# utiasASRL/mm_masking

Measured on AMD Instinct MI355X. Metric: scan-pairs/s (mask-CNN + 10-iter dICP fwd+bwd), higher is better.
Workload: dtype bf16; 1 GPU; BASELINE configs[2]: train_icp_weights step fwd+bwd, batch=32 per GPU, 10 dICP iters, point-to-plane Huber, dim=2; 400x3360 polar radar -> GO-CFAR + peaks + polar->Cartesian 640x640 -> U-Net (hand-written NHWC bf16 MFMA kernels, fp32 masters) -> dICP (fp32 points, fp64 normal equations) -> rot+trans+mask_pts loss -> Adam; batch_per_gpu=32, global_batch=32, scan_pts_pad=5120, map_pts=20000, map_pts_pad=20480, icp_iters=10, parallelism=dp1, scene_density=survey (SURVEY.md 8d: 3 500-5 000 valid scan points of 5 120)

## Files before the change

mm_masking_amd/csrc/mmk_unet.hip:

```cpp
#include <math.h>
#include <stdlib.h>

#include <algorithm>
#include <type_traits>

#include "mmk_common.h"
#include "mmk_unet_shared.h"

namespace {

using namespace mmku;

__device__ __forceinline__ unsigned cvt_pk_bf16(float lo, float hi)
{
    unsigned r;
    asm("v_cvt_pk_bf16_f32 %0, %1, %2" : "=v"(r) : "v"(lo), "v"(hi));
    return r;
}
__device__ __forceinline__ unsigned pk_relu_bf16(unsigned x)
{
    unsigned r;
    asm("v_pk_max_i16 %0, %1, 0" : "=v"(r) : "v"(x));
    return r;
}
// ... 670 lines not shown

    float bs8[8];
    if constexpr (C8) {
#pragma unroll
        for (int r = 0; r < 8; ++r) {
            bs8[r] = a.bias ? a.bias[r] : 0.f;
            asm volatile("" : "+v"(bs8[r]));
        }
    }
    const float dk = dp.inv_keep;
    const unsigned thr1pk = ((unsigned)(dp.thr_s - 1 < -32768 ? -32768 : dp.thr_s - 1) & 0xffffu) * 0x00010001u;
#pragma unroll
    for (int m = 0; m < MT; ++m)
#pragma unroll
        for (int r = 0; r < 4; ++r) bs[m][r] *= dk;
    if constexpr (C8) {
#pragma unroll
        for (int r = 0; r < 8; ++r) bs8[r] *= dk;
    }

    MMK_RING_LOAD(0);
    MMK_RING_LOAD(1);
    MMK_RING_SINKS();
    if constexpr (RD > 2) {
        MMK_RING_LOAD(2);
        MMK_RING_SINKS();
    }
    cur_pix0 = s_pix0[0]; cur_ty0 = s_ty0[0]; cur_tx0 = s_tx0[0];
    if constexpr (POOL) cur_pp0 = s_pp0[0];
    MMK_RING_STORE(0, 0);
    MMK_RING_LOAD(0);
    MMK_RING_SINKS();

    int k0 = 0;
    {
#define STAGE_CHECKED 1
#define STAGE_SLOT 0
#include "mmk_conv_ring_stage.inc"
#undef STAGE_SLOT
#define STAGE_SLOT 1
#include "mmk_conv_ring_stage.inc"
#undef STAGE_SLOT
        if constexpr (RD > 2) {
#define STAGE_SLOT 2
#include "mmk_conv_ring_stage.inc"
#undef STAGE_SLOT
        }
#undef STAGE_CHECKED
    }
    for (k0 = RD; k0 + RD <= nt_blk; k0 += RD) {
#define STAGE_CHECKED 0
#define STAGE_SLOT 0
#include "mmk_conv_ring_stage.inc"
#undef STAGE_SLOT
#define STAGE_SLOT 1
#include "mmk_conv_ring_stage.inc"
#undef STAGE_SLOT
        if constexpr (RD > 2) {
#define STAGE_SLOT 2
#include "mmk_conv_ring_stage.inc"
#undef STAGE_SLOT
        }
#undef STAGE_CHECKED
    }
    {
#define STAGE_CHECKED 1
#define STAGE_SLOT 0
#include "mmk_conv_ring_stage.inc"
#undef STAGE_SLOT
        if constexpr (RD > 2) {
#define STAGE_SLOT 1
#include "mmk_conv_ring_stage.inc"
#undef STAGE_SLOT
        }
#undef STAGE_CHECKED
    }
ring_done:;
#ifdef MMK_DEEP_STAMPS
    if (tid == 0) { stamp_lds[16 + 6] = __builtin_amdgcn_s_memtime(); stamp_lds[16 + 7] = __builtin_amdgcn_s_memrealtime(); }
    __syncthreads();
    if (g_deep_stamp_buf != nullptr && blockIdx.y == 0 && blockIdx.x < 4096 && tid == 0) {
        unsigned long long *life = g_deep_stamp_buf + (size_t)64 * (4 * MMK_STAMP_STAGES * 8) + (size_t)blockIdx.x * 2;
        life[0] = stamp_lds[8 + 7];
        life[1] = stamp_lds[16 + 7];
    }
    if (g_deep_stamp_buf != nullptr && blockIdx.y == 0 && blockIdx.x < 64)
        for (int i = tid; i < 4 * MMK_STAMP_STAGES * 8; i += CONV_THREADS)
            g_deep_stamp_buf[(size_t)blockIdx.x * (4 * MMK_STAMP_STAGES * 8) + i] = stamp_lds[i];
#endif
#undef MMK_RING_LOAD
#undef MMK_RING_STORE
}

template <int CK, int CM, int RD, bool EPI, int POOL = 0, bool C8 = false, bool POOLG = false>
int launch_conv_ring(const ConvArgs &a, hipStream_t st)
{
#ifdef MMK_DEEP_STAMPS
    const size_t smem = (((size_t)2 * HT * WT * lds_pitch(CK) + (size_t)ksteps(CK) * (CM / 16) * 512) * sizeof(bf16) + 15) / 16 * 16 +
                        (size_t)4 * MMK_STAMP_STAGES * 8 * sizeof(unsigned long long);
#else
    const size_t smem = ((size_t)2 * HT * WT * lds_pitch(CK) + (size_t)ksteps(CK) * (CM / 16) * 512) * sizeof(bf16);
#endif
    constexpr auto kernel = conv3x3_ring_kernel<CK, CM, RD, EPI, POOL, C8, POOLG>;
    int per_cu = 0;
    MMK_CHECK_HIP(blocks_per_cu<kernel>(CONV_THREADS, smem, 8, &per_cu));
    const int groups = (a.COUT + CM - 1) / CM;
    const XcdGrid g = xcd_grid(a.B, a.H, a.W, TH, TW, groups, per_cu);
    hipLaunchKernelGGL(kernel, dim3(8 * g.nb, groups), dim3(CONV_THREADS), smem, st, a, g.total, g.per_xcd);
    MMK_LAUNCH_CHECK();
    return MMK_OK;
}

inline bool use_c8_epilogue()
{
    static int v = -1;
    if (v < 0) {
        const char *e = getenv("MMK_CONV_C8");
        v = (e && e[0] == '0') ? 0 : 1;
    }
    return v == 1;
}

template <int CK, int CM>
int launch_conv_ring_epi(const ConvArgs &a, hipStream_t st)
{
    constexpr int RD = CK <= 16 ? 3 : 2;
    constexpr int RDE = 2;
    const bool epi = a.o1.relu_src || a.o1.accumulate || (a.o2.C > 0 && (a.o2.relu_src || a.o2.accumulate));
    if (a.x1_pool_arg != nullptr) {
        if constexpr (CK == 32 && CM == 32) {
            if (epi && a.pool_y == nullptr) return launch_conv_ring<CK, CM, RDE, true, 0, false, true>(a, st);
        }
        mmk::set_error("mmk_conv3x3: x1_pool_arg is not supported for this layer (CIN=%d COUT=%d)", a.CIN, a.COUT);
        return MMK_ERR_ARG;
    }
    if (a.pool_y != nullptr) {
        if constexpr (CK == CM && (CK == 16 || CK == 32)) {
            if (!epi && a.o2.C == 0)
                return a.pool_arg != nullptr ? launch_conv_ring<CK, CM, RD, false, 2>(a, st) : launch_conv_ring<CK, CM, RD, false, 1>(a, st);
        }
        mmk::set_error("mmk_conv3x3: pool_y is not supported for this layer (see mmk_conv3x3_pool_fusable)");
        return MMK_ERR_ARG;
    }
    if constexpr (CM == 16) {
        if (a.COUT == 8 && a.o2.C == 0 && use_c8_epilogue())
            return epi ? launch_conv_ring<CK, CM, RDE, true, false, true>(a, st) : launch_conv_ring<CK, CM, RD, false, false, true>(a, st);
    }
    return epi ? launch_conv_ring<CK, CM, RDE, true>(a, st) : launch_conv_ring<CK, CM, RD, false>(a, st);
}


constexpr int DEEP_THREADS = 512;

template <int BM, int NT>
struct DeepCfg {
    static constexpr int WM = BM >= 128 ? 2 : 1;
    static constexpr int WN = 8 / WM;
    static constexpr int MT = BM / 16 / WM;
    static constexpr int MTB = BM / 16;
    static constexpr int TH = WN, TWD = NT * 16;
    static constexpr int HT = TH + 2, WT = TWD + 2;
    static constexpr int CK = 32, PK = 48, NS = 9, GPP = 4;
    static constexpr int NIN = HT * WT * GPP;
    static constexpr int NW = NS * MTB * 64;
    static constexpr int RIN = (NIN + DEEP_THREADS - 1) / DEEP_THREADS;
    static constexpr int RW = (NW + DEEP_THREADS - 1) / DEEP_THREADS;
    static constexpr size_t IN_BYTES = (size_t)HT * WT * PK * sizeof(bf16), W_BYTES = (size_t)NW * 8 * sizeof(bf16);
    static constexpr size_t smem_core(int wchunks) { return IN_BYTES + (size_t)wchunks * W_BYTES + BM * sizeof(float); }
#ifdef MMK_DEEP_STAMPS
    static constexpr size_t smem(int wchunks) { return (smem_core(wchunks) + 15) / 16 * 16 + (size_t)8 * MMK_STAMP_STAGES * 8 * sizeof(unsigned long long); }
#else
    static constexpr size_t smem(int wchunks) { return smem_core(wchunks); }
#endif
};

template <int BM, int NT>
XcdGrid deep_grid(int B, int H, int W, int cout)
{
    return xcd_grid(B, H, W, DeepCfg<BM, NT>::TH, DeepCfg<BM, NT>::TWD, (cout + BM - 1) / BM, 1);
}

template <int BM, int NT, bool LK = false, bool SUBW = false, int ROLE = 0, bool WRES = false, bool POOLG = false>
__global__ __launch_bounds__(DEEP_THREADS) void conv3x3_deep_kernel(const ConvArgs a, int total_tiles, int tiles_per_xcd)
{
    using C = DeepCfg<BM, NT>;
    constexpr int MT = C::MT, MTB = C::MTB, PK = C::PK, WT = C::WT, HT = C::HT, GPP = C::GPP;
    constexpr int NIN = C::NIN, NW = C::NW, RIN = C::RIN, RW = C::RW, NS = C::NS;
    constexpr bool R_FWD = ROLE == 1, R_BWD = ROLE == 2;
    static_assert(!(WRES && SUBW), "resident weights: the kernel's own packing only");
    extern __shared__ __attribute__((aligned(16))) unsigned char smem[];
    bf16 *in_tile = reinterpret_cast<bf16 *>(smem);
    bf16 *w_lds = in_tile + HT * WT * PK;

    const int tid = threadIdx.x, lane = tid & 63, wv = tid >> 6;
    const int wm = wv / C::WN, wn = wv % C::WN;
    const int tiles_x = (a.W + C::TWD - 1) / C::TWD, tiles_y = (a.H + C::TH - 1) / C::TH;
    const int tpi = tiles_x * tiles_y;
    const int group = blockIdx.y;
    const int nchunk = a.CIN / 32;
    const int wchunks = WRES ? nchunk : 1;

    const int xcd = blockIdx.x & 7, nb = gridDim.x >> 3;
    const int t_begin = xcd * tiles_per_xcd;
    const int t_end = (t_begin + tiles_per_xcd < total_tiles) ? t_begin + tiles_per_xcd : total_tiles;
    int tile = t_begin + (blockIdx.x >> 3);
    if (tile >= t_end) return;

    constexpr int RWL = WRES ? 0 : RW;
    constexpr int PHT = C::TH / 2 + 2, PWT = C::TWD / 2 + 2, NPIN = PHT * PWT * GPP;
    constexpr int NRIN = POOLG ? (NPIN + DEEP_THREADS - 1) / DEEP_THREADS : RIN;
    u32x4 rin[NRIN], rw[RW];
    unsigned rcd[POOLG ? NRIN : 1];
    const int Hp = a.H >> 1, Wp = a.W >> 1;
    int g_dy[RIN], g_dx[RIN], g_c[RIN], g_pix[RIN];
#pragma unroll
    for (int i = 0; i < RIN; ++i) {
        int g = tid + i * DEEP_THREADS;
        g = g < NIN ? g : NIN - 1;
        const int pix = g / GPP;
        g_dy[i] = pix / WT - 1;
        g_dx[i] = pix % WT - 1;
        g_c[i] = (g % GPP) * 8;
        g_pix[i] = (pix / WT) * a.W + pix % WT;
        if constexpr (POOLG) {
            int gp = tid + i * DEEP_THREADS;
            gp = gp < NPIN ? gp : NPIN - 1;
            const int pp = gp / GPP;
            g_dy[i] = pp / PWT - 1;
            g_dx[i] = pp % PWT - 1;
            g_c[i] = (gp % GPP) * 8;
            g_pix[i] = g_dy[i] * Wp + g_dx[i];
        }
    }
    const bf16 *ld_base = nullptr;
    int ld_xc = 0, ld_ty0 = 0, ld_tx0 = 0;
    const u32x4 *ld_w = nullptr;
    const unsigned *ld_code = nullptr;
    int ld_moff = 0;
    auto set_stage = [&](int t, int chunk) {
        const int b = t / tpi, tr = t - b * tpi;
        const int tyi = tr / tiles_x;
        ld_tx0 = (tr - tyi * tiles_x) * C::TWD;
        ld_ty0 = tyi * C::TH;
        const int c0 = chunk * 32;
        const bool in1 = c0 < a.C1;
        const bf16 *xb = in1 ? a.x1 : a.x2;
        ld_xc = in1 ? a.C1 : a.C2;
        const int cb = in1 ? c0 : c0 - a.C1;
        const long org = POOLG ? ((long)b * Hp + (ld_ty0 >> 1)) * Wp + (ld_tx0 >> 1)
                               : ((long)b * a.H + ld_ty0 - 1) * a.W + ld_tx0 - 1;
        ld_base = xb + org * ld_xc + cb;
        if constexpr (POOLG) ld_code = a.x1_pool_arg + ((org * ld_xc + cb) >> 3);
        if constexpr (SUBW) {
            const int pm = a.wpack_mtb, per = pm / MTB;
            ld_w = reinterpret_cast<const u32x4 *>(a.wpack + ((size_t)((group / per) * nchunk + chunk)) * NS * pm * 512);
            ld_moff = (group % per) * MTB;
        } else {
            ld_w = reinterpret_cast<const u32x4 *>(a.wpack + ((size_t)(group * nchunk + chunk)) * NW * 8);
        }
    };
    auto issue_in = [&](int i) {
        if constexpr (POOLG) {
            const bool ok = (unsigned)((ld_ty0 >> 1) + g_dy[i]) < (unsigned)Hp && (unsigned)((ld_tx0 >> 1) + g_dx[i]) < (unsigned)Wp;
            const int off = g_pix[i] * ld_xc + g_c[i];
            rin[i] = *(ok ? reinterpret_cast<const u32x4 *>(ld_base + off) : &g_zero16);
            rcd[i] = *(ok ? ld_code + (off >> 3) : reinterpret_cast<const unsigned *>(&g_zero16));
            return;
        }
        const bool ok = (unsigned)(ld_ty0 + g_dy[i]) < (unsigned)a.H && (unsigned)(ld_tx0 + g_dx[i]) < (unsigned)a.W;
        const unsigned off = (unsigned)(g_pix[i] * ld_xc + g_c[i]);
        const u32x4 *sp = ok ? reinterpret_cast<const u32x4 *>(ld_base + off) : &g_zero16;
        rin[i] = *sp;
    };
    auto issue_w = [&](int i) {
        int g = tid + i * DEEP_THREADS;
        g = g < NW ? g : NW - 1;
        if constexpr (SUBW) rw[i] = ld_w[((g / (MTB * 64)) * a.wpack_mtb + ld_moff) * 64 + g % (MTB * 64)];
        else rw[i] = ld_w[g];
    };
    auto write_in = [&]() {
        if constexpr (POOLG) {
#pragma unroll
            for (int i = 0; i < NRIN; ++i) {
                const int g = tid + i * DEEP_THREADS;
                const int r0 = 2 * g_dy[i] + 1, c0 = 2 * g_dx[i] + 1;
                poolg_write(in_tile + (r0 * WT + c0) * PK + g_c[i], PK, WT * PK, r0, c0, HT, WT, g < NPIN, rin[i], rcd[i], a.x1_pool_scale);
            }
            return;
        }
#pragma unroll
        for (int i = 0; i < RIN; ++i) {
            const int g = tid + i * DEEP_THREADS;
            if (g < NIN) *reinterpret_cast<u32x4 *>(in_tile + (size_t)(g / GPP) * PK + (g % GPP) * 8) = rin[i];
        }
    };
    auto write_w = [&](int slot) {
#pragma unroll
        for (int i = 0; i < RW; ++i) {
            const int g = tid + i * DEEP_THREADS;
            if (g < NW) reinterpret_cast<u32x4 *>(w_lds + (size_t)slot * NW * 8)[g] = rw[i];
        }
    };

    const DropoutParams dp = dropout_params(a.drop_p);
    float *bias_lds = reinterpret_cast<float *>(w_lds + (size_t)wchunks * NW * 8);
    if (tid < BM) {
        int c = group * BM + tid;
        if constexpr (SUBW) {
            const int pm = a.wpack_mtb, per = pm / MTB, m_off = (group % per) * MTB;
            c = (group / per) * (pm * 16) + (m_off / 4) * 64 + 16 * (tid / (4 * MT)) + 4 * (m_off % 4) + tid % (4 * MT);
        }
        const float bz = (a.bias && c < a.COUT) ? a.bias[c] : 0.f;
        bias_lds[tid] = R_FWD ? bz * dp.inv_keep : bz;
    }
    f32x4 acc[MT][NT];
    auto reset_acc = [&]() {
#pragma unroll
        for (int m = 0; m < MT; ++m)
#pragma unroll
            for (int n = 0; n < NT; ++n) acc[m][n] = f32x4{0.f, 0.f, 0.f, 0.f};
    };
    reset_acc();

    constexpr bool lk = LK;
    const bf16 *b_base = in_tile + ((size_t)(wn * WT + (lane & 15))) * PK + 8 * (lane >> 4);
    const bf16 *a_base0 = w_lds + ((size_t)(wm * MT) * 64 + lane) * 8;

    int chunk = 0;
#ifdef MMK_DEEP_STAMPS
    unsigned long long *stamp_lds = reinterpret_cast<unsigned long long *>(smem + (C::smem_core(wchunks) + 15) / 16 * 16);
    int stamp_stage = 0;
    for (int i = tid; i < 8 * MMK_STAMP_STAGES * 8; i += DEEP_THREADS) stamp_lds[i] = 0ull;
#endif
    if constexpr (WRES) {
        for (int ck = 0; ck < nchunk; ++ck) {
            set_stage(tile, ck);
#pragma unroll
            for (int i = 0; i < RW; ++i) issue_w(i);
            write_w(ck);
        }
    }
    set_stage(tile, 0);
#pragma unroll
    for (int i = 0; i < NRIN; ++i) issue_in(i);
    if constexpr (!WRES) {
#pragma unroll
        for (int i = 0; i < RW; ++i) issue_w(i);
        write_w(0);
    }
    write_in();
    __syncthreads();

    constexpr int NCH = 4 * MT;
    constexpr int LW = NCH >= 8 ? 8 : 4;
    typedef __attribute__((ext_vector_type(LW))) __bf16 bfl;
    constexpr int NP = NCH / LW;

    while (true) {
        MMK_STAMP(0);
        int ntile = tile, nck = chunk + 1;
        if (nck == nchunk) {
            nck = 0;
            ntile = tile + nb;
        }
        const bool has_next = ntile < t_end;
        set_stage(has_next ? ntile : tile, nck);
        const bf16 *a_base = a_base0 + (WRES ? (size_t)chunk * NW * 8 : (size_t)0);
        MMK_STAMP(1);
#pragma unroll
        for (int s = 0; s < NS; ++s) {
            const int ty = s / 3, tx = s % 3;
            bf16x8 bf[NT];
#pragma unroll
            for (int n = 0; n < NT; ++n)
                bf[n] = *reinterpret_cast<const bf16x8 *>(b_base + ((size_t)(ty * WT + n * 16 + tx)) * PK);
#pragma unroll
            for (int m = 0; m < MT; ++m) {
                const bf16x8 af = *reinterpret_cast<const bf16x8 *>(a_base + ((size_t)(s * MTB + m) * 64) * 8);
#pragma unroll
                for (int n = 0; n < NT; ++n) acc[m][n] = __builtin_amdgcn_mfma_f32_16x16x32_bf16(af, bf[n], acc[m][n], 0, 0, 0);
            }
#pragma unroll
            for (int j = s; j < NRIN + RWL; j += NS) {
                if (j < NRIN) issue_in(j);
                else issue_w(j - NRIN);
            }
            __builtin_amdgcn_sched_barrier(0x38F);
        }
        MMK_STAMP(2);
        auto deliver_and_write = [&]() {
#pragma unroll
            for (int i = 0; i < NRIN; ++i) asm volatile("" : "+v"(rin[i]));
            if constexpr (POOLG) {
#pragma unroll
                for (int i = 0; i < NRIN; ++i) asm volatile("" : "+v"(rcd[i]));
            }
#pragma unroll
            for (int i = 0; i < RWL; ++i) asm volatile("" : "+v"(rw[i]));
            MMK_STAMP(4);
            if (has_next) {
                __syncthreads();
                MMK_STAMP(5);
                write_in();
                if constexpr (!WRES) write_w(0);
            }
            MMK_STAMP(6);
        };
        if (chunk != nchunk - 1) {
            MMK_STAMP(3);
            deliver_and_write();
        } else {
            const int b = tile / tpi, tr = tile - b * tpi;
            const int tyi = tr / tiles_x;
            const int tx0 = (tr - tyi * tiles_x) * C::TWD, yy = tyi * C::TH + wn;
            int lv = lane;
            asm volatile("" : "+v"(lv));
            const int g4 = lv >> 4;
            int c0, e_bias_at;
            if constexpr (SUBW) {
                const int pm = a.wpack_mtb, per = pm / MTB, m_off = (group % per) * MTB;
                c0 = (group / per) * (pm * 16) + (m_off / 4) * 64 + 16 * g4 + 4 * (m_off % 4);
                e_bias_at = NCH * g4;
            } else {
                c0 = group * BM + wm * (16 * MT) + NCH * g4;
                e_bias_at = wm * (16 * MT) + NCH * g4;
            }
            const bool e_on = c0 < a.COUT;
            const bool firstp = c0 < a.o1.C;
            bf16 *const o_y = firstp ? a.o1.y : a.o2.y;
            const bf16 *const o_src = firstp ? a.o1.relu_src : a.o2.relu_src;
            const int o_C = firstp ? a.o1.C : a.o2.C;
            const bool e_acc = (firstp ? a.o1.accumulate : a.o2.accumulate) != 0;
            const float e_scale = firstp ? a.o1.scale : a.o2.scale;
            const int cl = firstp ? c0 : c0 - a.o1.C;
            const int e_x0 = tx0 + (lv & 15);
            const long p0 = ((long)b * a.H + yy) * a.W + e_x0;
            const unsigned e_e0 = (unsigned)p0 * (unsigned)a.COUT + (unsigned)c0 + a.hash_base;
            bf16 *const e_y0 = o_y + p0 * o_C + cl;
            const int e_step = 16 * o_C;
            const bool e_row_ok = yy < a.H;
            const bool e_src = o_src != nullptr;
            const bf16 *const e_pf0 = e_src ? o_src + p0 * o_C + cl : (e_acc ? (const bf16 *)e_y0 : nullptr);
            bfl opnd[R_BWD ? NT : 1][NP];
            auto fetch_operands = [&]() {
#pragma unroll
                for (int n = 0; n < NT; ++n) {
                    const bool okp = e_on && e_pf0 != nullptr && e_row_ok && e_x0 + n * 16 < a.W;
                    const bf16 *pp = okp ? e_pf0 + n * e_step : reinterpret_cast<const bf16 *>(g_zero32);
#pragma unroll
                    for (int k = 0; k < NP; ++k) opnd[R_BWD ? n : 0][k] = *reinterpret_cast<const bfl *>(pp + k * LW);
                }
            };
            if constexpr (R_BWD) fetch_operands();
            if (e_on) {
                if constexpr (R_FWD) {
                    float bk[NCH];
#pragma unroll
                    for (int k = 0; k < NCH; k += 4) {
                        const f32x4 t = *reinterpret_cast<const f32x4 *>(bias_lds + e_bias_at + k);
                        bk[k] = t[0]; bk[k + 1] = t[1]; bk[k + 2] = t[2]; bk[k + 3] = t[3];
                    }
                    const float kf = dp.inv_keep;
                    const int t1s = (int)dp.thr - 32768 - 1;
                    const unsigned t1 = (unsigned)(t1s < -32768 ? -32768 : t1s) & 0xffffu;
                    const unsigned thr1 = t1 | (t1 << 16);
                    const bool drop = dp.thr != 0u;
#pragma unroll
                    for (int n = 0; n < NT; ++n) {
                        const bool okp = e_row_ok && e_x0 + n * 16 < a.W;
                        unsigned hw[MT][2];
#pragma unroll
                        for (int m = 0; m < MT; ++m) hw[m][0] = hw[m][1] = 0x7fff7fffu;
                        if (drop) {
#pragma unroll
                            for (int m = 0; m < MT; ++m)
                                dropout_words(a.seed, e_e0 + (unsigned)n * (16u * (unsigned)a.COUT) + 4u * m, hw[m][0], hw[m][1]);
                        }
                        unsigned pk[NCH / 2];
#pragma unroll
                        for (int m = 0; m < MT; ++m)
#pragma unroll
                            for (int hlf = 0; hlf < 2; ++hlf) {
                                const float t0 = __builtin_fmaf(acc[m][n][2 * hlf], kf, bk[4 * m + 2 * hlf]);
                                const float t1f = __builtin_fmaf(acc[m][n][2 * hlf + 1], kf, bk[4 * m + 2 * hlf + 1]);
                                pk[2 * m + hlf] = pk_relu_bf16(cvt_pk_bf16(t0, t1f)) & pk_keep_mask(hw[m][hlf], thr1);
                            }
                        bf16 *const dst = okp ? e_y0 + n * e_step : reinterpret_cast<bf16 *>(g_sink32);
                        if constexpr (NCH >= 8) {
#pragma unroll
                            for (int k = 0; k < NCH / 2; k += 4)
                                *reinterpret_cast<u32x4 *>(dst + 2 * k) = (u32x4){pk[k], pk[k + 1], pk[k + 2], pk[k + 3]};
                        } else {
                            *reinterpret_cast<unsigned long long *>(dst) = ((unsigned long long)pk[1] << 32) | pk[0];
                        }
                        __builtin_amdgcn_sched_barrier(0);
                    }
                } else {
                    float bv[NCH];
                    if constexpr (!R_BWD) {
#pragma unroll
                        for (int k = 0; k < NCH; k += 4) {
                            const f32x4 t = *reinterpret_cast<const f32x4 *>(bias_lds + e_bias_at + k);
                            bv[k] = t[0]; bv[k + 1] = t[1]; bv[k + 2] = t[2]; bv[k + 3] = t[3];
                        }
                    }
                    const bool o_accf = !e_src && e_acc;
#pragma unroll
                    for (int n = 0; n < NT; ++n) {
                        const bool okp = e_row_ok && e_x0 + n * 16 < a.W;
                        float v[NCH];
#pragma unroll
                        for (int m = 0; m < MT; ++m)
#pragma unroll
                            for (int r = 0; r < 4; ++r) {
                                float t = acc[m][n][r];
                                if constexpr (!R_BWD) {
                                    t += bv[4 * m + r];
                                    if (a.relu) t = lk ? act_leaky(t, a.slope) : fmaxf(t, 0.f);
                                }
                                v[4 * m + r] = t;
                            }
                        if constexpr (!R_BWD) {
                            if (dp.thr != 0u) {
#pragma unroll
                                for (int m = 0; m < MT; ++m) {
                                    float sc[4];
                                    dropout_scale4(a.seed, e_e0 + (unsigned)n * (16u * (unsigned)a.COUT) + 4u * m, dp, sc);
#pragma unroll
                                    for (int r = 0; r < 4; ++r) v[4 * m + r] = lk ? drop_leaky(v[4 * m + r], sc[r]) : v[4 * m + r] * sc[r];
                                }
                            }
                        }
                        bf16 *const dst0 = e_y0 + n * e_step;
                        if constexpr (R_BWD) {
                            if (e_pf0 != nullptr && okp) {
                                if (!o_accf) {
#pragma unroll
                                    for (int k = 0; k < NCH; k += LW) {
                                        const bfl sv = opnd[n][k / LW];
#pragma unroll
                                        for (int r = 0; r < LW; ++r) v[k + r] = ((float)sv[r] > 0.f) ? v[k + r] * e_scale : 0.f;
                                    }
                                } else {
#pragma unroll
                                    for (int k = 0; k < NCH; k += LW) {
                                        const bfl ov = opnd[n][k / LW];
#pragma unroll
                                        for (int r = 0; r < LW; ++r) v[k + r] += (float)ov[r];
                                    }
                                }
                            }
                        } else {
                            if (e_src && okp) {
                                const bf16 *sp = e_pf0 + n * e_step;
#pragma unroll
                                for (int k = 0; k < NCH; k += LW) {
                                    const bfl sv = *reinterpret_cast<const bfl *>(sp + k);
#pragma unroll
                                    for (int r = 0; r < LW; ++r)
                                        v[k + r] = lk ? v[k + r] * bwd_factor_leaky((float)sv[r], e_scale, a.slope)
                                                      : (((float)sv[r] > 0.f) ? v[k + r] * e_scale : 0.f);
                                }
                            }
                            if (e_acc && okp) {
#pragma unroll
                                for (int k = 0; k < NCH; k += LW) {
                                    const bfl ov = *reinterpret_cast<const bfl *>(dst0 + k);
#pragma unroll
                                    for (int r = 0; r < LW; ++r) v[k + r] += (float)ov[r];
                                }
                            }
                        }
                        if (R_BWD || okp) {
                            bf16 *const dst = (R_BWD && !okp) ? reinterpret_cast<bf16 *>(g_sink32) : dst0;
                            if constexpr (NCH >= 8) {
#pragma unroll
                                for (int k = 0; k < NCH; k += 8) {
                                    bf16x8 o8;
#pragma unroll
                                    for (int r = 0; r < 8; ++r) o8[r] = (bf16)v[k + r];
                                    *reinterpret_cast<bf16x8 *>(dst + k) = o8;
                                }
                            } else {
                                bf16x4 o4;
#pragma unroll
                                for (int r = 0; r < 4; ++r) o4[r] = (bf16)v[r];
                                *reinterpret_cast<bf16x4 *>(dst) = o4;
                            }
                        }
                    }
                }
            }
            reset_acc();
            MMK_STAMP(3);
            deliver_and_write();
        }
        if (!has_next) break;
        __syncthreads();
        MMK_STAMP(7);
#ifdef MMK_DEEP_STAMPS
        ++stamp_stage;
#endif
        tile = ntile;
        chunk = nck;
    }
#ifdef MMK_DEEP_STAMPS
    __syncthreads();
    if (g_deep_stamp_buf != nullptr && blockIdx.y == 0 && blockIdx.x < 64)
        for (int i = tid; i < 8 * MMK_STAMP_STAGES * 8; i += DEEP_THREADS)
            g_deep_stamp_buf[(size_t)blockIdx.x * (8 * MMK_STAMP_STAGES * 8) + i] = stamp_lds[i];
#endif
}

template <int BM, int NT, bool LK = false, bool SUBW = false, int ROLE = 0, bool WRES = false, bool POOLG = false>
int launch_conv_deep(const ConvArgs &a, hipStream_t st)
{
    using C = DeepCfg<BM, NT>;
    constexpr auto kernel = conv3x3_deep_kernel<BM, NT, LK, SUBW, ROLE, WRES, POOLG>;
    MMK_CHECK_HIP(raise_lds_limit<kernel>(true, 160 * 1024));
    const size_t smem = C::smem(WRES ? a.CIN / 32 : 1);
    MMK_REQUIRE(smem <= (size_t)160 * 1024, "mmk_conv3x3: %zu bytes of LDS for CIN=%d COUT=%d", smem, a.CIN, a.COUT);
    const XcdGrid g = deep_grid<BM, NT>(a.B, a.H, a.W, a.COUT);
    hipLaunchKernelGGL(kernel, dim3(8 * g.nb, (a.COUT + BM - 1) / BM), dim3(DEEP_THREADS), smem, st, a, g.total, g.per_xcd);
    MMK_LAUNCH_CHECK();
    return MMK_OK;
}

template <int BM, int NT>
bool deep_weights_fit(int cin) { return DeepCfg<BM, NT>::smem(cin / 32) <= (size_t)160 * 1024; }

template <class F>
int with_deep_cfg(int BM, bool narrow, F &&f)
{
    return with_int<16, 32, 64, 128>(BM, [&](auto M) {
        return narrow ? f(M, std::integral_constant<int, 3>{}) : f(M, std::integral_constant<int, 5>{});
    });
}

int deep_rounds(int B, int H, int W, int cout, int BM, bool narrow, int *tiles_per_image)
{
    return with_deep_cfg(BM, narrow, [&](auto M, auto NT) {
        const XcdGrid g = deep_grid<M(), NT()>(B, H, W, cout);
        if (tiles_per_image) *tiles_per_image = g.tiles;
        return g.rounds();
    });
}

int dispatch_conv_deep_plain(const ConvArgs &a, hipStream_t st);

int dispatch_conv_deep(const ConvArgs &a, hipStream_t st)
{
    const int BM = conv_cm(a.CIN, a.COUT);
    const bool narrow = a.W <= 48;
    const char *split_env = getenv("MMK_CONV_SPLIT");
    const bool split_on = !(split_env && split_env[0] == '0');
    int tpi = 0;
    const bool forward_role = a.relu != 0 && a.o1.relu_src == nullptr && a.o2.relu_src == nullptr && !a.o1.accumulate && !a.o2.accumulate;
    if (split_on && forward_role && a.slope == 0.f && (BM == 64 || BM == 128) && a.COUT % 32 == 0 && a.pool_y == nullptr && a.wpack_mtb == 0 &&
        deep_rounds(a.B, a.H, a.W, a.COUT, BM, narrow, &tpi) == 2) {
        const int groups = (a.COUT + BM - 1) / BM, nb = std::max(1, 32 / groups);
        const int Bm = (8 * nb) / tpi;
        const int Bt = a.B - Bm;
        const bool under_filled = (long)a.B * tpi * groups * 10 < (long)256 * 2 * 7;
        if (Bm >= 1 && Bt >= 1 && under_filled && deep_rounds(Bm, a.H, a.W, a.COUT, BM, narrow, nullptr) == 1 &&
            deep_rounds(Bt, a.H, a.W, a.COUT, 32, narrow, nullptr) == 1 && (a.o1.C % 32 == 0) && (a.o2.C % 32 == 0)) {
            ConvArgs m = a;
            m.B = Bm;
            int rc = dispatch_conv_deep_plain(m, st);
            if (rc != MMK_OK) return rc;
            ConvArgs t = a;
            const size_t px = (size_t)Bm * a.H * a.W;
            t.B = Bt;
            t.x1 = a.x1 + px * a.C1;
            if (a.x2) t.x2 = a.x2 + px * a.C2;
            auto adv = [&](ConvOutPart &o) {
                if (o.y) o.y += px * o.C;
                if (o.relu_src) o.relu_src += px * o.C;
            };
            adv(t.o1);
            adv(t.o2);
            t.hash_base = a.hash_base + (unsigned)(px * a.COUT);
            t.wpack_mtb = BM / 16;
            return narrow ? launch_conv_deep<32, 3, false, true, 1>(t, st) : launch_conv_deep<32, 5, false, true, 1>(t, st);
        }
    }
    return dispatch_conv_deep_plain(a, st);
}

int dispatch_conv_deep_plain(const ConvArgs &a, hipStream_t st)
{
    const bool any_src = a.o1.relu_src != nullptr || (a.o2.C > 0 && a.o2.relu_src != nullptr);
    const bool any_acc = a.o1.accumulate != 0 || (a.o2.C > 0 && a.o2.accumulate != 0);
    const bool both1 = a.o1.relu_src != nullptr && a.o1.accumulate != 0, both2 = a.o2.C > 0 && a.o2.relu_src != nullptr && a.o2.accumulate != 0;
    const int role = (a.relu != 0 && !any_src && !any_acc) ? 1
                   : ((a.relu == 0 && a.bias == nullptr && dropout_params(a.drop_p).thr == 0u && !both1 && !both2) ? 2 : 0);
    const int rc = with_deep_cfg(conv_cm(a.CIN, a.COUT), a.W <= 48, [&](auto M, auto N) -> int {
        constexpr int BM = M(), NT = N();
        constexpr bool WRES = BM <= 64;
        const bool resident = WRES && a.wpack_mtb == 0 && deep_weights_fit<BM, NT>(a.CIN);
        if (a.slope > 0.f) return launch_conv_deep<BM, NT, true>(a, st);
        if (a.x1_pool_arg != nullptr) {
            if constexpr (BM >= 64) {
                if (role == 2 && a.wpack_mtb == 0) {
                    if (resident) return launch_conv_deep<BM, NT, false, false, 2, WRES, true>(a, st);
                    if (BM > 64) return launch_conv_deep<BM, NT, false, false, 2, false, true>(a, st);
                }
            }
            mmk::set_error("mmk_conv3x3: x1_pool_arg is not supported for this layer (CIN=%d COUT=%d)", a.CIN, a.COUT);
            return MMK_ERR_ARG;
        }
        if constexpr (BM >= 32) {
            if (role == 1) return resident ? launch_conv_deep<BM, NT, false, false, 1, WRES>(a, st) : launch_conv_deep<BM, NT, false, false, 1>(a, st);
            if (role == 2) return resident ? launch_conv_deep<BM, NT, false, false, 2, WRES>(a, st) : launch_conv_deep<BM, NT, false, false, 2>(a, st);
        }
        return launch_conv_deep<BM, NT>(a, st);
    });
    if (rc != NO_KERNEL) return rc;
    mmk::set_error("mmk_conv3x3: unsupported channel counts CIN=%d COUT=%d", a.CIN, a.COUT);
    return MMK_ERR_ARG;
}

bool pool_fusable(int cin, int cout, int B, int H, int W)
{
    const bool fits32 = (size_t)B * H * W * (size_t)std::max(cin, cout) < ((size_t)1 << 31);
    return cin == cout && (cin == 16 || cin == 32) && fits32 && H >= 2 && W >= 2;
}

template <class F>
int with_thin_shape(int CK, int CM, F &&f)
{
    return with_int<8, 16, 32>(CK, [&](auto K) {
        return with_int<16, 32, 64>(CM, [&](auto M) {
            if constexpr (K() == 32 && M() == 64) return NO_KERNEL;
            else return f(K, M);
        });
    });
}

int dispatch_conv(const ConvArgs &a, hipStream_t st)
{
    if (a.pool_y != nullptr && (a.slope > 0.f || !pool_fusable(a.CIN, a.COUT, a.B, a.H, a.W))) {
        mmk::set_error("mmk_conv3x3: pool_y is not supported for this layer (see mmk_conv3x3_pool_fusable)");
        return MMK_ERR_ARG;
    }
    if (a.x1_pool_arg != nullptr && (a.slope > 0.f || a.C2 != 0 || a.H < 2 || a.W < 2)) {
        mmk::set_error("mmk_conv3x3: x1_pool_arg needs the ReLU network, a single input and H, W >= 2");
        return MMK_ERR_ARG;
    }
    if (conv_is_deep(a.CIN, a.COUT)) {
        if (a.o2.C > 0 && conv_cm(a.CIN, a.COUT) >= 64 && a.o1.C % 16 != 0) {
            mmk::set_error("mmk_conv3x3: output split %d+%d: layers of >= 64 output channels split at multiples of 16", a.o1.C, a.o2.C);
            return MMK_ERR_ARG;
        }
        return dispatch_conv_deep(a, st);
    }
    const int CK = conv_ck(a.CIN), CM = conv_cm(a.CIN, a.COUT);
    if (a.x1_pool_arg != nullptr && !(a.CIN == 32 && CM == 32 && (size_t)a.B * a.H * a.W * 32 < ((size_t)1 << 31))) {
        mmk::set_error("mmk_conv3x3: x1_pool_arg is not supported for this layer (CIN=%d COUT=%d)", a.CIN, a.COUT);
        return MMK_ERR_ARG;
    }
    const bool fits32 = (size_t)a.B * a.H * a.W * (size_t)std::max(a.CIN, a.COUT) < ((size_t)1 << 31);
    const bool ring = a.CIN == CK && CM <= 32 && fits32;
    const int rc = with_thin_shape(CK, CM, [&](auto K, auto M) -> int {
        if (a.slope > 0.f) return launch_conv<K(), M(), true>(a, st);
        if constexpr (M() <= 32) {
            if (ring) return launch_conv_ring_epi<K(), M()>(a, st);
        }
        return launch_conv<K(), M()>(a, st);
    });
    if (rc != NO_KERNEL) return rc;
    mmk::set_error("mmk_conv3x3: unsupported channel counts CIN=%d COUT=%d", a.CIN, a.COUT);
    return MMK_ERR_ARG;
}


typedef __attribute__((ext_vector_type(2))) int i32x2;
typedef __attribute__((ext_vector_type(4))) int i32x4;

__device__ __forceinline__ unsigned lds_addr(const void *p)
{
    return (unsigned)(size_t)(__attribute__((address_space(3))) const void *)p;
}

__device__ __forceinline__ i32x2 tr_read(unsigned addr)
{
    i32x2 v;
    asm volatile("ds_read_b64_tr_b16 %0, %1" : "=v"(v) : "v"(addr) : "memory");
    return v;
}

template <int OFF>
__device__ __forceinline__ i32x2 tr_read_o(unsigned addr)
{
    static_assert(OFF >= 0 && OFF < 65536, "ds offset field is 16 bits");
    i32x2 v;
    asm volatile("ds_read_b64_tr_b16 %0, %1 offset:%2" : "=v"(v) : "v"(addr), "n"(OFF) : "memory");
    return v;
}

__device__ __forceinline__ bf16x8 frag_from(i32x2 lo, i32x2 hi)
{
    i32x4 t = {lo.x, lo.y, hi.x, hi.y};
    return __builtin_bit_cast(bf16x8, t);
}

struct WgradArgs {
    const bf16 *x1, *x2;
    int C1, C2;
    const bf16 *g;
    int B, H, W, CIN, COUT;
    float *partials;
    int acc_partials;
    const unsigned *g_arg = nullptr;
    float g_scale = 1.f;
};

template <int CK, int CM, bool G8, bool POOLG = false>
__global__ __launch_bounds__(CONV_THREADS) void conv3x3_wgrad_kernel(const WgradArgs a)
{
    constexpr int MT = CM / 16;
    constexpr int NTT = (CK >= 16) ? 9 * (CK / 16) : 5;
    constexpr int NTW = (NTT + 3) / 4;
    extern __shared__ __attribute__((aligned(16))) unsigned char smem[];
    constexpr int PK = wg_pitch(CK);
    constexpr int GCOLS = G8 ? 8 : CM;
    constexpr int PG = wg_pitch(GCOLS);
    bf16 *x_tile = reinterpret_cast<bf16 *>(smem);
    bf16 *g_tile = x_tile + (HT * WT + 8) * PK;

    const int tid = threadIdx.x, lane = tid & 63;
    const int wv = __builtin_amdgcn_readfirstlane(tid >> 6);
    const int chunk = blockIdx.y, group = blockIdx.z;
    const int tiles_x = (a.W + TW - 1) / TW, tiles_y = (a.H + TH - 1) / TH;
    const int tpi = tiles_x * tiles_y;
    const int total_tiles = tpi * a.B;
    const int i16 = lane & 15, g4 = lane >> 4, q = i16 >> 2, pp = i16 & 3;

    f32x4 acc[MT][NTW];
    f32x4 accb[MT];
#pragma unroll
    for (int m = 0; m < MT; ++m) {
        accb[m] = (f32x4){0.f, 0.f, 0.f, 0.f};
#pragma unroll
        for (int n = 0; n < NTW; ++n) acc[m][n] = (f32x4){0.f, 0.f, 0.f, 0.f};
    }
    bf16x8 ones;
#pragma unroll
    for (int j = 0; j < 8; ++j) ones[j] = (bf16)1.0f;
// ... 2834 lines not shown
```

Before: 3431 pairs/s.

## Fold two image rows into each wave's pixel fragments for narrow deep convs

Adds a FOLD variant of the deep 3x3 conv kernel for 128-channel layers with width 33-40. Each wave covers two output rows packed into five 16-pixel fragments, so the tile is 2*WN rows by 40 columns. Without folding, a row of about 40 pixels is padded to 48 and the extra MFMA columns are wasted. The dispatcher enables the fold by default (env switch MMK_CONV_FOLD), and the batch-split path gains a tail variant. The costs are a more complex gather address per fragment and extra template instantiations.

```diff
diff --git a/mm_masking_amd/csrc/mmk_unet.hip b/mm_masking_amd/csrc/mmk_unet.hip
--- a/mm_masking_amd/csrc/mmk_unet.hip
+++ b/mm_masking_amd/csrc/mmk_unet.hip
@@ -846,13 +846,14 @@
 
 constexpr int DEEP_THREADS = 512;
 
-template <int BM, int NT>
+template <int BM, int NT, bool FOLD = false>
 struct DeepCfg {
+    static_assert(!FOLD || (BM == 128 && NT == 5), "folded rows: 128 output channels per block, five fragments per row pair");
     static constexpr int WM = BM >= 128 ? 2 : 1;
     static constexpr int WN = 8 / WM;
     static constexpr int MT = BM / 16 / WM;
     static constexpr int MTB = BM / 16;
-    static constexpr int TH = WN, TWD = NT * 16;
+    static constexpr int TH = FOLD ? 2 * WN : WN, TWD = FOLD ? NT * 8 : NT * 16;
     static constexpr int HT = TH + 2, WT = TWD + 2;
     static constexpr int CK = 32, PK = 48, NS = 9, GPP = 4;
     static constexpr int NIN = HT * WT * GPP;
@@ -868,16 +869,17 @@
 #endif
 };
 
-template <int BM, int NT>
+template <int BM, int NT, bool FOLD = false>
 XcdGrid deep_grid(int B, int H, int W, int cout)
 {
-    return xcd_grid(B, H, W, DeepCfg<BM, NT>::TH, DeepCfg<BM, NT>::TWD, (cout + BM - 1) / BM, 1);
-}
-
-template <int BM, int NT, bool LK = false, bool SUBW = false, int ROLE = 0, bool WRES = false, bool POOLG = false>
+    return xcd_grid(B, H, W, DeepCfg<BM, NT, FOLD>::TH, DeepCfg<BM, NT, FOLD>::TWD, (cout + BM - 1) / BM, 1);
+}
+
+template <int BM, int NT, bool LK = false, bool SUBW = false, int ROLE = 0, bool WRES = false, bool POOLG = false, bool FOLD = false>
 __global__ __launch_bounds__(DEEP_THREADS) void conv3x3_deep_kernel(const ConvArgs a, int total_tiles, int tiles_per_xcd)
 {
-    using C = DeepCfg<BM, NT>;
+    using C = DeepCfg<BM, NT, FOLD>;
+    static_assert(!FOLD || (!LK && !SUBW && !WRES && !POOLG && ROLE != 0), "folded rows: the plain forward and data-gradient roles");
     constexpr int MT = C::MT, MTB = C::MTB, PK = C::PK, WT = C::WT, HT = C::HT, GPP = C::GPP;
     constexpr int NIN = C::NIN, NW = C::NW, RIN = C::RIN, RW = C::RW, NS = C::NS;
     constexpr bool R_FWD = ROLE == 1, R_BWD = ROLE == 2;
@@ -1018,6 +1020,16 @@
 
     constexpr bool lk = LK;
     const bf16 *b_base = in_tile + ((size_t)(wn * WT + (lane & 15))) * PK + 8 * (lane >> 4);
+    const bf16 *b_fold[FOLD ? NT : 1];
+    if constexpr (FOLD) {
+#pragma unroll
+        for (int n = 0; n < NT; ++n) {
+            int q = n * 16 + (lane & 15);
+            q = q < 2 * a.W ? q : 2 * a.W - 1;
+            const int r = q >= a.W ? 1 : 0;
+            b_fold[n] = in_tile + ((size_t)((2 * wn + r) * WT + q - r * a.W)) * PK + 8 * (lane >> 4);
+        }
+    }
     const bf16 *a_base0 = w_lds + ((size_t)(wm * MT) * 64 + lane) * 8;
 
     int chunk = 0;
@@ -1066,8 +1078,10 @@
             const int ty = s / 3, tx = s % 3;
             bf16x8 bf[NT];
 #pragma unroll
-            for (int n = 0; n < NT; ++n)
-                bf[n] = *reinterpret_cast<const bf16x8 *>(b_base + ((size_t)(ty * WT + n * 16 + tx)) * PK);
+            for (int n = 0; n < NT; ++n) {
+                if constexpr (FOLD) bf[n] = *reinterpret_cast<const bf16x8 *>(b_fold[n] + ((size_t)(ty * WT + tx)) * PK);
+                else bf[n] = *reinterpret_cast<const bf16x8 *>(b_base + ((size_t)(ty * WT + n * 16 + tx)) * PK);
+            }
 #pragma unroll
             for (int m = 0; m < MT; ++m) {
                 const bf16x8 af = *reinterpret_cast<const bf16x8 *>(a_base + ((size_t)(s * MTB + m) * 64) * 8);
@@ -1106,7 +1120,7 @@
         } else {
             const int b = tile / tpi, tr = tile - b * tpi;
             const int tyi = tr / tiles_x;
-            const int tx0 = (tr - tyi * tiles_x) * C::TWD, yy = tyi * C::TH + wn;
+            const int tx0 = (tr - tyi * tiles_x) * C::TWD, yy = tyi * C::TH + (FOLD ? 2 * wn : wn);
             int lv = lane;
             asm volatile("" : "+v"(lv));
             const int g4 = lv >> 4;
@@ -1133,13 +1147,18 @@
             bf16 *const e_y0 = o_y + p0 * o_C + cl;
             const int e_step = 16 * o_C;
             const bool e_row_ok = yy < a.H;
+            const int e_qlim = yy + 1 < a.H ? 2 * a.W : (e_row_ok ? a.W : 0);
+            auto pix_ok = [&](int n) {
+                if constexpr (FOLD) return e_x0 + n * 16 < e_qlim;
+                else return e_row_ok && e_x0 + n * 16 < a.W;
+            };
             const bool e_src = o_src != nullptr;
             const bf16 *const e_pf0 = e_src ? o_src + p0 * o_C + cl : (e_acc ? (const bf16 *)e_y0 : nullptr);
             bfl opnd[R_BWD ? NT : 1][NP];
             auto fetch_operands = [&]() {
 #pragma unroll
                 for (int n = 0; n < NT; ++n) {
-                    const bool okp = e_on && e_pf0 != nullptr && e_row_ok && e_x0 + n * 16 < a.W;
+                    const bool okp = e_on && e_pf0 != nullptr && pix_ok(n);
                     const bf16 *pp = okp ? e_pf0 + n * e_step : reinterpret_cast<const bf16 *>(g_zero32);
 #pragma unroll
                     for (int k = 0; k < NP; ++k) opnd[R_BWD ? n : 0][k] = *reinterpret_cast<const bfl *>(pp + k * LW);
@@ -1161,7 +1180,7 @@
                     const bool drop = dp.thr != 0u;
 #pragma unroll
                     for (int n = 0; n < NT; ++n) {
-                        const bool okp = e_row_ok && e_x0 + n * 16 < a.W;
+                        const bool okp = pix_ok(n);
                         unsigned hw[MT][2];
 #pragma unroll
                         for (int m = 0; m < MT; ++m) hw[m][0] = hw[m][1] = 0x7fff7fffu;
@@ -1201,7 +1220,7 @@
                     const bool o_accf = !e_src && e_acc;
 #pragma unroll
                     for (int n = 0; n < NT; ++n) {
-                        const bool okp = e_row_ok && e_x0 + n * 16 < a.W;
+                        const bool okp = pix_ok(n);
                         float v[NCH];
 #pragma unroll
                         for (int m = 0; m < MT; ++m)
@@ -1306,15 +1325,15 @@
 #endif
 }
 
-template <int BM, int NT, bool LK = false, bool SUBW = false, int ROLE = 0, bool WRES = false, bool POOLG = false>
+template <int BM, int NT, bool LK = false, bool SUBW = false, int ROLE = 0, bool WRES = false, bool POOLG = false, bool FOLD = false>
 int launch_conv_deep(const ConvArgs &a, hipStream_t st)
 {
-    using C = DeepCfg<BM, NT>;
-    constexpr auto kernel = conv3x3_deep_kernel<BM, NT, LK, SUBW, ROLE, WRES, POOLG>;
+    using C = DeepCfg<BM, NT, FOLD>;
+    constexpr auto kernel = conv3x3_deep_kernel<BM, NT, LK, SUBW, ROLE, WRES, POOLG, FOLD>;
     MMK_CHECK_HIP(raise_lds_limit<kernel>(true, 160 * 1024));
     const size_t smem = C::smem(WRES ? a.CIN / 32 : 1);
     MMK_REQUIRE(smem <= (size_t)160 * 1024, "mmk_conv3x3: %zu bytes of LDS for CIN=%d COUT=%d", smem, a.CIN, a.COUT);
-    const XcdGrid g = deep_grid<BM, NT>(a.B, a.H, a.W, a.COUT);
+    const XcdGrid g = deep_grid<BM, NT, FOLD>(a.B, a.H, a.W, a.COUT);
     hipLaunchKernelGGL(kernel, dim3(8 * g.nb, (a.COUT + BM - 1) / BM), dim3(DEEP_THREADS), smem, st, a, g.total, g.per_xcd);
     MMK_LAUNCH_CHECK();
     return MMK_OK;
@@ -1331,8 +1350,13 @@
     });
 }
 
-int deep_rounds(int B, int H, int W, int cout, int BM, bool narrow, int *tiles_per_image)
-{
+int deep_rounds(int B, int H, int W, int cout, int BM, bool narrow, bool fold, int *tiles_per_image)
+{
+    if (fold && BM == 128) {
+        const XcdGrid g = deep_grid<128, 5, true>(B, H, W, cout);
+        if (tiles_per_image) *tiles_per_image = g.tiles;
+        return g.rounds();
+    }
     return with_deep_cfg(BM, narrow, [&](auto M, auto NT) {
         const XcdGrid g = deep_grid<M(), NT()>(B, H, W, cout);
         if (tiles_per_image) *tiles_per_image = g.tiles;
@@ -1340,27 +1364,46 @@
     });
 }
 
-int dispatch_conv_deep_plain(const ConvArgs &a, hipStream_t st);
+int dispatch_conv_deep_plain(const ConvArgs &a, hipStream_t st, bool fold);
+
+int deep_role(const ConvArgs &a)
+{
+    const bool any_src = a.o1.relu_src != nullptr || (a.o2.C > 0 && a.o2.relu_src != nullptr);
+    const bool any_acc = a.o1.accumulate != 0 || (a.o2.C > 0 && a.o2.accumulate != 0);
+    const bool both1 = a.o1.relu_src != nullptr && a.o1.accumulate != 0, both2 = a.o2.C > 0 && a.o2.relu_src != nullptr && a.o2.accumulate != 0;
+    return (a.relu != 0 && !any_src && !any_acc) ? 1
+         : ((a.relu == 0 && a.bias == nullptr && dropout_params(a.drop_p).thr == 0u && !both1 && !both2) ? 2 : 0);
+}
+
+bool deep_folds(const ConvArgs &a)
+{
+    const char *fold_env = getenv("MMK_CONV_FOLD");
+    if (fold_env && fold_env[0] == '0') return false;
+    return conv_cm(a.CIN, a.COUT) == 128 && a.W >= 33 && a.W <= 40 && a.slope == 0.f && a.x1_pool_arg == nullptr && a.wpack_mtb == 0 &&
+           deep_role(a) != 0;
+}
 
 int dispatch_conv_deep(const ConvArgs &a, hipStream_t st)
 {
     const int BM = conv_cm(a.CIN, a.COUT);
-    const bool narrow = a.W <= 48;
+    const bool narrow = a.W <= 48, fold = deep_folds(a);
     const char *split_env = getenv("MMK_CONV_SPLIT");
     const bool split_on = !(split_env && split_env[0] == '0');
     int tpi = 0;
     const bool forward_role = a.relu != 0 && a.o1.relu_src == nullptr && a.o2.relu_src == nullptr && !a.o1.accumulate && !a.o2.accumulate;
     if (split_on && forward_role && a.slope == 0.f && (BM == 64 || BM == 128) && a.COUT % 32 == 0 && a.pool_y == nullptr && a.wpack_mtb == 0 &&
-        deep_rounds(a.B, a.H, a.W, a.COUT, BM, narrow, &tpi) == 2) {
+        deep_rounds(a.B, a.H, a.W, a.COUT, BM, narrow, fold, &tpi) == 2) {
         const int groups = (a.COUT + BM - 1) / BM, nb = std::max(1, 32 / groups);
         const int Bm = (8 * nb) / tpi;
         const int Bt = a.B - Bm;
         const bool under_filled = (long)a.B * tpi * groups * 10 < (long)256 * 2 * 7;
-        if (Bm >= 1 && Bt >= 1 && under_filled && deep_rounds(Bm, a.H, a.W, a.COUT, BM, narrow, nullptr) == 1 &&
-            deep_rounds(Bt, a.H, a.W, a.COUT, 32, narrow, nullptr) == 1 && (a.o1.C % 32 == 0) && (a.o2.C % 32 == 0)) {
+        const bool head_ok = Bm >= 1 && Bt >= 1 && under_filled && deep_rounds(Bm, a.H, a.W, a.COUT, BM, narrow, fold, nullptr) == 1;
+        const bool tail32 = head_ok && deep_rounds(Bt, a.H, a.W, a.COUT, 32, narrow, false, nullptr) == 1 && (a.o1.C % 32 == 0) && (a.o2.C % 32 == 0);
+        const bool tail_own = head_ok && !tail32 && fold && deep_rounds(Bt, a.H, a.W, a.COUT, BM, narrow, false, nullptr) == 1;
+        if (tail32 || tail_own) {
             ConvArgs m = a;
             m.B = Bm;
-            int rc = dispatch_conv_deep_plain(m, st);
+            int rc = dispatch_conv_deep_plain(m, st, fold);
             if (rc != MMK_OK) return rc;
             ConvArgs t = a;
             const size_t px = (size_t)Bm * a.H * a.W;
@@ -1374,20 +1417,20 @@
             adv(t.o1);
             adv(t.o2);
             t.hash_base = a.hash_base + (unsigned)(px * a.COUT);
+            if (tail_own) return dispatch_conv_deep_plain(t, st, false);
             t.wpack_mtb = BM / 16;
             return narrow ? launch_conv_deep<32, 3, false, true, 1>(t, st) : launch_conv_deep<32, 5, false, true, 1>(t, st);
         }
     }
-    return dispatch_conv_deep_plain(a, st);
-}
-
-int dispatch_conv_deep_plain(const ConvArgs &a, hipStream_t st)
-{
-    const bool any_src = a.o1.relu_src != nullptr || (a.o2.C > 0 && a.o2.relu_src != nullptr);
-    const bool any_acc = a.o1.accumulate != 0 || (a.o2.C > 0 && a.o2.accumulate != 0);
-    const bool both1 = a.o1.relu_src != nullptr && a.o1.accumulate != 0, both2 = a.o2.C > 0 && a.o2.relu_src != nullptr && a.o2.accumulate != 0;
-    const int role = (a.relu != 0 && !any_src && !any_acc) ? 1
-                   : ((a.relu == 0 && a.bias == nullptr && dropout_params(a.drop_p).thr == 0u && !both1 && !both2) ? 2 : 0);
+    return dispatch_conv_deep_plain(a, st, fold);
+}
+
+int dispatch_conv_deep_plain(const ConvArgs &a, hipStream_t st, bool fold)
+{
+    const int role = deep_role(a);
+    if (fold)
+        return role == 1 ? launch_conv_deep<128, 5, false, false, 1, false, false, true>(a, st)
+                         : launch_conv_deep<128, 5, false, false, 2, false, false, true>(a, st);
     const int rc = with_deep_cfg(conv_cm(a.CIN, a.COUT), a.W <= 48, [&](auto M, auto N) -> int {
         constexpr int BM = M(), NT = N();
         constexpr bool WRES = BM <= 64;
```

Result: faster. 3481 pairs/s (median of 6 runs) (+1.5%).
